# getanteon/alaz

Measured on AMD Instinct MI355X. Metric: L7 edge-events/s ingested->scored service-map, higher is better.
Workload: dtype u64; 1 GPU; C3 device-resident replay: 10000 pods / 5000 services / 1000000 edges, 10000000 HTTP l7 events per window already in HBM, 2-layer SAGE + MLP score, partitioned K1 (variant 0, 8-byte records, 512 partitions); 2-batch HBM ring (value excludes PCIe: see end_to_end with --full); events_per_window=10000000, layers=2, windows_in_flight=1, parallelism=1 GPU

## Files before the change

### alaz_amd/csrc/servicegraph.hip

```cpp
#include <hip/hip_runtime.h>
#include <hip/hip_ext.h>

#include <algorithm>
#include <cmath>
#include <cstdio>
#include <cstring>
#include <chrono>
#include <condition_variable>
#include <thread>
#include <mutex>
#include <string>
#include <unordered_map>
#include <vector>

#include <dlfcn.h>

#include "join_host.hpp"
#include "sg_plan.hpp"
#include "sg_kernels.h"
#include "sg_sel.h"
#include "sg_trend.h"
#include "sg_node_trend.h"
#include "sg_rank.h"
#include "sg_incident.h"
// ... 141 lines not shown
                    u32* blk = nullptr; u32* stage = nullptr; u32* stage_idx = nullptr; std::vector<sg_group_edge*> rows; std::vector<u64*> count;
                    std::vector<u32*> row_group, perm; std::vector<char> valid; hipEvent_t ev = nullptr; bool pending = false;
                    std::vector<u32> h_map; u32* h_up = nullptr; hipEvent_t up_ev = nullptr; bool up_pending = false; u32 dirty_lo = 0, dirty_hi = 0;
                    u32 hi_group = 0; } grp;
    Baseline<sg_edge_trend> gtrend;
    Vanished gvanished;
    IdxSel<sg_group_edge> gsel;
    Rollup<sgplan::GroupNodesPlan> gnodes;
    Baseline<sg_node_trend> gntrend;
    NSel gnsel;
    Rank<sgplan::GroupRankPlan> grank;
    Incidents<sgplan::GroupIncidentPlan> ginc;
};

namespace {

sg_engine::WinSlot& work(sg_engine* e) { return e->slots[e->cur]; }
int ran_slot(const sg_engine* e) { return e->last.slot >= 0 ? e->last.slot : e->cur; }
sg_engine::WinSlot& ran(sg_engine* e) { return e->slots[ran_slot(e)]; }

#define HIP_TRY(e, call)                                                                       \
    do {                                                                                       \
        hipError_t _r = (call);                                                                \
        if (_r != hipSuccess) {                                                                \
            (e)->err = std::string(#call) + ": " + hipGetErrorString(_r);                      \
            return _r == hipErrorOutOfMemory ? SG_ENOMEM : SG_ENODEV;                          \
        }                                                                                      \
    } while (0)

template <typename T>
int dev_alloc(sg_engine* e, T** p, size_t n, int fill = 0) {
    void* q = nullptr;
    size_t bytes = std::max<size_t>(n, 1) * sizeof(T);
    constexpr size_t kArenaMax = (size_t)32 << 20, kArenaChunk = (size_t)256 << 20, kArenaAlign = 4096;
    if (e->plan.arena_on && bytes < kArenaMax) {
        const size_t need = (bytes + kArenaAlign - 1) & ~(kArenaAlign - 1);
        if (need > e->arena_left) {
            void* c = nullptr;
            HIP_TRY(e, hipMalloc(&c, kArenaChunk));
            e->allocs.push_back(c);
            e->arena_base = static_cast<char*>(c); e->arena_left = kArenaChunk;
        }
        q = e->arena_base; e->arena_base += need; e->arena_left -= need;
    } else {
        HIP_TRY(e, hipMalloc(&q, bytes));
        e->allocs.push_back(q);
    }
    HIP_TRY(e, hipMemsetAsync(q, fill, bytes, e->slots[0].stream));
    *p = (T*)q;
    return SG_OK;
}

hipStream_t pick(sg_engine* e, void* s) { return s ? (hipStream_t)s : work(e).stream; }
hipStream_t pick_ran(sg_engine* e, void* s) { return s ? (hipStream_t)s : e->last.slot >= 0 ? e->last.stream : work(e).stream; }

hipEvent_t get_event(sg_engine* e) {
    if (!e->ev_pool.empty()) { hipEvent_t v = e->ev_pool.back(); e->ev_pool.pop_back(); return v; }
    hipEvent_t v; hipEventCreate(&v); return v;
}

struct Timed {
    sg_engine* e; hipStream_t s; TimingRec r; bool on;
    Timed(sg_engine* e_, hipStream_t s_, int kernel) : e(e_), s(s_), on(e_ && ((e_->timing >> kernel) & 1u)) {
        if (on) { r.kernel = kernel; r.a = get_event(e); r.b = get_event(e); hipEventRecord(r.a, s); }
    }
    ~Timed() { if (on) { hipEventRecord(r.b, s); e->trecs.push_back(r); } }
};

static_assert(sgplan::kK1bWarmU == K1B_WARM_U, "sg_plan.hpp's copy of pass B's warm U");
constexpr int k4_threads(int fi, bool proj, bool split) { return split ? (proj ? 512 : 256) : (fi == 32 ? 1024 : 512); }
template <class FnT, const auto& Keys> struct Family { typedef FnT Fn; static constexpr auto& keys = Keys; };
struct K1aWide : Family<K1aFn, sgplan::kK1aWideKeys> { template <size_t I> static Fn at() { constexpr auto k = keys[I]; return k1a_partition<(bool)k[0], (bool)k[1], (bool)k[2]>; } };
struct K1aTile : Family<K1aFn, sgplan::kK1aTileKeys> { template <size_t I> static Fn at() { constexpr auto k = keys[I]; return k1a_tile_partition<k[0], (bool)k[1], k[2]>; } };
struct K1aTeam : Family<K1aFn, sgplan::kK1aTeamKeys> { template <size_t I> static Fn at() { constexpr auto k = keys[I]; return k1a_team_partition<k[0], (bool)k[1], 2, 1024, k[2]>; } };
struct K1bMerge : Family<K1bFn, sgplan::kK1bMergeKeys> { template <size_t I> static Fn at() {
    constexpr auto k = keys[I]; if constexpr (k[2]) return k1b_merge<k[0], (bool)k[1]>; else return k1b_merge_wide<k[0], (bool)k[1]>; } };
struct K1bStream : Family<K1bFn, sgplan::kK1bStreamKeys> { template <size_t I> static Fn at() {
    constexpr auto k = keys[I]; if constexpr (k[4]) return k1b_stream_merge<k[0], k[1], (bool)k[2], k[3]>; else return k1b_stream_merge_wide<k[0], k[1], (bool)k[2], k[3]>; } };
struct K4Layer : Family<K4LayerFn, sgplan::kK4LayerKeys> { template <size_t I> static Fn at() {
    constexpr auto k = keys[I]; return k4_sage_layer<k[0], (bool)k[1], (bool)k[2], k4_threads(k[0], k[2], k[3]), (bool)k[3]>; } };
constexpr K2RowptrFn kK2Rowptr[2] = {k2_rowptr<K2_RP_ROWS, false>, k2_rowptr<K2_RP_ROWS_DH, true>};
constexpr K4GatherFn kK4Gather[2] = {k4_gather<32>, k4_gather<64>};
constexpr K5ProjFn kK5Proj[2] = {k5_node_proj<false>, k5_node_proj<true>};
constexpr K5ScoreFn kK5Score[2] = {k5_edge_score<false>, k5_edge_score<true>};
template <class F, size_t... I>
const std::array<typename F::Fn, sizeof...(I)>& kernel_table(std::index_sequence<I...>) {
    static const std::array<typename F::Fn, sizeof...(I)> t{{F::template at<I>()...}};
    return t;
}
template <class F> const auto& kernel_table() { return kernel_table<F>(std::make_index_sequence<F::keys.size()>{}); }
template <class F, class... A>
typename F::Fn kernel_of(bool& ok, A... args) {
    const int i = sgplan::find_key(F::keys, sgplan::Key<sizeof...(A)>{{(int)args...}});
    if (i < 0) ok = false;
    return i < 0 ? nullptr : kernel_table<F>()[i];
}
template <class... K>
hipError_t lds_limit(size_t bytes, K... kernels) {
    for (const void* f : {reinterpret_cast<const void*>(kernels)...}) {
        const hipError_t r = hipFuncSetAttribute(f, hipFuncAttributeMaxDynamicSharedMemorySize, (int)bytes);
        if (r != hipSuccess) return r;
    }
    return hipSuccess;
}
template <class F>
hipError_t lds_limit_all(size_t bytes) { hipError_t r = hipSuccess; for (const auto f : kernel_table<F>()) if (r == hipSuccess) r = lds_limit(bytes, f); return r; }

int plan_pass_a(sg_engine* e) {
    sgplan::PassA pa = e->pa;
    if (!sgplan::plan_pass_a(e->plan, e->jt.l1_entries, e->jt.blocks_bytes(), e->ov, &pa)) { e->err = "K1 pass A: the join tables' level 1 and the piece counters do not fit a CU's LDS (fewer partitions / IP blocks needed)"; return SG_ENOSPC; }
    const sgplan::PassAKernel k = sgplan::choose_pass_a(e->plan, pa, e->cfg);
    bool ok = true;
    const K1aFn f = k.family == sgplan::K1A_TEAM ? kernel_of<K1aTeam>(ok, k.l2, k.sharded, k.pb)
                  : k.family == sgplan::K1A_TILE ? kernel_of<K1aTile>(ok, k.l2, k.sharded, k.nsub) : kernel_of<K1aWide>(ok, k.l2, k.sharded, k.hist);
    if (!ok) { e->err = "K1 pass A: the library holds no kernel for family " + std::to_string(k.family) + ", level 2 mode " + std::to_string(k.l2); return SG_ENODEV; }
    e->pa = pa; e->kn.k1a = k; e->fn.k1a = f;
    return SG_OK;
}
int resolve_kernels(sg_engine* e) {
    const sgplan::Kernels& k = e->kn;
    sg_engine::Fns& f = e->fn;
    bool ok = true;
    if (k.k1b_family == sgplan::K1B_STREAM) {
        f.k1b = kernel_of<K1bStream>(ok, k.k1b_u, k.k1b_spt, k.k1b_pack, 0, k.k1b_share);
        if (k.k1b_warm) f.k1b_try = kernel_of<K1bStream>(ok, sgplan::kK1bWarmU, k.k1b_spt, k.k1b_pack, 1, k.k1b_share);
        if (k.k1b_warm) f.k1b_cold = kernel_of<K1bStream>(ok, sgplan::kK1bWarmU, k.k1b_spt, k.k1b_pack, 2, k.k1b_share);
    } else if (k.k1b_family == sgplan::K1B_MERGE) f.k1b = kernel_of<K1bMerge>(ok, k.k1b_u, k.k1b_hist, k.k1b_share);
    f.k2_rowptr = kK2Rowptr[k.k2_dh]; f.k5_proj = kK5Proj[k.k5_mfma];
    for (int w = 0; w < 2; w++) for (int pj = 0; pj < 2; pj++) f.k4_layer[w][pj] = kernel_of<K4Layer>(ok, w ? 64 : 32, k.k4_mfma, pj, k.k4_split);
    if (!ok) { e->err = "the library holds no kernel for one of the plan's choices (sg_plan.hpp choose_kernels)"; return SG_ENODEV; }
    return SG_OK;
}


void join_view(const sg_engine* e, Dev& d) {
    d.jl1mask = e->jt.l1_entries - 1;
    d.jl2_words = e->jt.use_blocks ? e->jt.blocks_used * 256u : 0u;
    d.ck_n = e->jt.ck_n;
    d.jstage_bytes = (u32)((size_t)e->jt.l1_entries * 8 + (e->pa.l2_in_lds ? e->jt.blocks_bytes() : 0));
    d.jl2_in_lds = e->pa.l2_in_lds ? 1u : 0u;
    d.k1a_ct = e->pa.k1a_ct;
}

int sync_tables(sg_engine* e, hipStream_t s) {
    sgjoin::Table& jt = e->jt;
    if (!jt.need_full && jt.dirty.empty()) return SG_OK;
    for (hipStream_t ks : e->k1_streams) if (ks != s) { HIP_TRY(e, hipEventRecord(e->k1_ev, ks)); HIP_TRY(e, hipStreamWaitEvent(s, e->k1_ev, 0)); }
    e->k1_streams.clear();
    if (jt.rebuilds == 0 && !jt.rebuild()) { e->err = "join table build failed: raise max_ips"; return SG_ENOSPC; }
    if (jt.need_full) {
        HIP_TRY(e, hipEventSynchronize(e->blob_ev));
        std::memcpy(e->h_blob, jt.blob, (size_t)jt.L.words * 4);
        HIP_TRY(e, hipMemcpyAsync(e->d_blob, e->h_blob, (size_t)jt.L.words * 4, hipMemcpyHostToDevice, s));
        HIP_TRY(e, hipEventRecord(e->blob_ev, s));
        jt.uploaded_full();
        e->st.join_full_uploads++;
    } else {
        std::vector<std::pair<u32, u32>> log;
        jt.take_dirty(log);
        std::unordered_map<u32, u32> last;
        last.reserve(log.size() * 2);
        for (auto& kv : log) last[kv.first] = kv.second;
        const int slot = e->upd_next; e->upd_next = (slot + 1) % kUpdSlots;
        HIP_TRY(e, hipEventSynchronize(e->upd_ev[slot]));
        u32 n = 0;
        for (auto& kv : last) e->h_upd[slot][n++] = make_uint2(kv.first, kv.second);
        HIP_TRY(e, hipMemcpyAsync(e->d_upd[slot], e->h_upd[slot], (size_t)n * sizeof(uint2), hipMemcpyHostToDevice, s));
// ... 589 lines not shown
    a.groups = e->grp.rows[e->cur]; a.gcount = e->grp.count[e->cur];
    a.max_groups = P.max_groups; a.gk = (u32)P.gk; a.hi_group = e->grp.hi_group; a.nc = P.nc;
    return a;
}
int launch_group_nodes(sg_engine* e, hipStream_t s) {
    GroupNodesArgs a = group_nodes_view(e);
    return launch_rollup(e, e->gnodes, e->gnodes.plan, s, a, a.nd, k16_out, k16_in_part, k16_count, k16_write);
}
static_assert(sgplan::kGrpRankThreads == K17_THREADS && sgplan::kGrpRankRangeRows == K17_NR && sgplan::kGrpRankMaxWgs == K17_MAX_WGS &&
              sgplan::kGrpRankNodeRows == K17_NODE_ROWS && K17_THREADS % K17_NODE_ROWS == 0 &&
              2 * sgplan::kGrpRankRangeRows * 8 <= sgplan::kLdsBytes, "plan_group_rank sizes the launches of sg_group_rank.h");
int launch_group_rank(sg_engine* e, hipStream_t s) {
    const sgplan::GroupRankPlan& P = e->grank.plan;
    GroupRankArgs a{};
    a.g = group_nodes_view(e);
    a.pos_wgs = P.pos_wgs; a.pos = e->grank.pos; a.w = e->grank.w;
    return launch_ranking(e, workload_space(e), P, s, a, [&](dim3 nt) {
        hipLaunchKernelGGL(k17_pos, dim3(P.pos_wgs), nt, 0, s, a);
        hipLaunchKernelGGL(k17_prep, dim3(P.prep_wgs), nt, 0, s, a);
    }, k17_edge<true>, k17_node<true, false>, k17_edge<false>, k17_node<false, false>, k17_node<false, true>);
}
void free_group_rank(sg_engine* e) { free_stage(e->grank); }
static_assert(sgplan::kGrpIncThreads == K18_THREADS && sgplan::kGrpIncMaxWgs == K18_MAX_WGS && sgplan::kGrpIncSlots == K12_SLOTS &&
              sgplan::kIncKeysBytes == sizeof(K12Keys), "plan_group_incidents sizes the launches of sg_group_incident.h");
int launch_group_incidents(sg_engine* e, hipStream_t s) {
    const sgplan::GroupIncidentPlan& P = e->ginc.plan;
    GroupIncArgs a{};
    a.g = group_nodes_view(e);
    a.pos = e->ginc.pos; a.esrc = e->ginc.esrc;
    return launch_grouping(e, workload_space(e), P, s, a, a.g.nd, P.fold_wgs, k18_init, k18_hook, k18_label, k18_number, k18_nodes, k18_rows, k18_finish);
}
void free_group_incidents(sg_engine* e) { free_stage(e->ginc); }
template <class Row>
void free_idxsel(sg_engine::IdxSel<Row>& s) {
    if (s.mem || s.h_n) hipDeviceSynchronize();
    if (s.mem) hipFree(s.mem);
    if (s.h_n) hipHostFree(s.h_n);
    if (s.ev) hipEventDestroy(s.ev);
    s = sg_engine::IdxSel<Row>{};
}
void free_group_nodes(sg_engine* e) {
    free_group_incidents(e);
    free_group_rank(e);
    free_idxsel(e->gnsel);
    free_baseline(e->gntrend);
    free_stage(e->gnodes);
}

void free_groups(sg_engine* e) {
    free_group_nodes(e);
    free_edge_trend(group_edge_space(e));
    sg_engine::Groups& x = e->grp;
    if (x.mem) hipDeviceSynchronize();
    if (x.h_up) hipHostFree(x.h_up);
    if (x.up_ev) hipEventDestroy(x.up_ev);
    free_stage(x);
}

void free_incidents(sg_engine* e) {
    free_tracks(e);
    free_stage(e->inc);
}

void free_nodes(sg_engine* e) {
    free_incidents(e);
    free_rank(e);
    free_baseline(e->ntrend);
    free_stage(e->nodes);
}

void drop_incidents(sg_engine* e, const EdgeSpace& es) {
    const NodeSpace ns = es.nodes(e);
    if (ns.inc->on && ns.inc->p.by != SG_SEL_SCORE) ns.inc_off(e);
}

int do_score(sg_engine* e, hipStream_t s, bool proj_done, bool fuse_reset, bool* did_reset) {
    const Dev& d = work(e).d;
    if (!e->have_w) { e->err = "sg_load_weights not called"; return SG_ESTATE; }
    const float* Wh = e->d_W + layer_offset(e->cfg.layers);
    const bool fr = fuse_reset && d.variant == 0;
    {
        Timed t(e, s, 5);
        if (!(proj_done && d.world == 1)) hipLaunchKernelGGL(e->fn.k5_proj, dim3(grid_for(d.ncap, 16)), dim3(256), 0, s, d, d.h[e->cfg.layers], Wh);
        hipLaunchKernelGGL(kK5Score[fr], dim3((int)e->plan.k5_grid), dim3(256), 0, s, d, Wh);
    }
    if (did_reset) *did_reset = fr;
    HIP_TRY(e, hipGetLastError());
    if (const int rc = note_w_read(e, s)) return rc;
    if (e->trend.on) { const int rc = launch_trend(e, s); if (rc) return rc; }
    if (e->nodes.on) {
        if (const int rc = launch_nodes(e, s)) return rc;
        if (e->ntrend.on) { if (const int rc = launch_node_trend(e, node_space(e), s, k10_count, k10_write)) return rc; }
        if (e->rank.on) { if (const int rc = launch_rank(e, s)) return rc; }
        if (e->inc.on) { if (const int rc = launch_incidents(e, s)) return rc; }
        if (e->trk.on) { if (const int rc = launch_tracks(e, s)) return rc; }
    }
    if (e->grp.on) {
        if (const int rc = launch_groups(e, s)) return rc;
        if (e->gtrend.on) { if (const int rc = launch_group_trend(e, s)) return rc; }
        if (e->gnodes.on) {
            if (const int rc = launch_group_nodes(e, s)) return rc;
            if (e->gntrend.on) { if (const int rc = launch_node_trend(e, workload_space(e), s, k16_tcount, k16_twrite)) return rc; }
            if (e->grank.on) { if (const int rc = launch_group_rank(e, s)) return rc; }
            if (e->ginc.on) { if (const int rc = launch_group_incidents(e, s)) return rc; }
        }
    }
    return SG_OK;
}

int do_reset(sg_engine* e, hipStream_t s) {
    sg_engine::WinSlot& w = work(e);
    hipLaunchKernelGGL(k_reset_window, dim3(grid_for(std::max<u64>((u64)w.d.ncap * SG_NODE_STAT_SUM_WORDS, e->plan.obcap), 256, 512)), dim3(256), 0, s, w.d);
    HIP_TRY(e, hipGetLastError());
    w.closed = false;
    w.events_in = 0;
    return SG_OK;
}

void window_timed_end(sg_engine* e, hipStream_t s) {
    if (!e->win_ta) return;
    TimingRec r; r.kernel = 10; r.a = e->win_ta; r.b = get_event(e);
    hipEventRecord(r.b, s);
    e->trecs.push_back(r);
    e->win_ta = nullptr;
}

void account_window(sg_engine* e) {
    sg_engine::WinSlot& w = work(e);
    const size_t E = (size_t)e->h_ctr[C_N_EDGES];
    sg_stats& st = e->st;
    st.windows++;
    st.last_window_events = e->h_ctr[C_N_EVENTS];
    st.last_window_edges = E;
    st.last_window_nodes = e->h_ctr[C_N_NODES];
    st.events_dropped_src += e->h_ctr[C_DROPPED_SRC];
    st.events_dropped_cap += e->h_ctr[C_DROPPED_CAP];
    st.events_misrouted += e->h_ctr[C_MISROUTED];
    {
        const u64 h = e->h_ctr[C_HALO_OVF];
        st.halo_overflow += h - w.halo_ovf_seen;
        w.halo_ovf_seen = h;
    }
    st.alive_in += e->h_ctr[C_ALIVE_SEEN];
    st.alive_dropped += e->h_ctr[C_ALIVE_DROPPED];
    st.last_window_new_edges = 0;
    if (w.d.warm && w.plain) st.windows_plain++;
    else if (w.d.warm) {
        const bool cold = e->h_ctr[C_LAST_COLD] != 0;
        if (cold) st.windows_cold++; else st.windows_warm++;
        if (!cold && e->h_ctr[C_LAST_DELTA]) { st.windows_delta++; st.last_window_new_edges = e->h_ctr[C_LAST_DELTA]; }
    }
    if (e->h_ctr[C_N_EVENTS]) {
        st.last_window_tmin_ms = (int64_t)((e->first_user - (e->first_kernel - e->h_ctr[C_TMIN_NS])) / 1000000ull);
        st.last_window_tmax_ms = (int64_t)((e->first_user - (e->first_kernel - e->h_ctr[C_TMAX_NS])) / 1000000ull);
    } else { st.last_window_tmin_ms = st.last_window_tmax_ms = 0; }
}

int view_reserve(sg_engine* e, size_t E) {
    if (E <= e->h_rows_cap) return SG_OK;
    if (e->h_rows_old) { hipHostFree(e->h_rows_old); e->h_rows_old = nullptr; }
    e->h_rows_old = e->h_rows; e->h_rows = nullptr; e->h_rows_cap = 0;
    const size_t want = std::min<size_t>(next_pow2(std::max<size_t>(E, 1024)), std::max<size_t>(e->cfg.max_edges, E));
    HIP_TRY(e, hipHostMalloc((void**)&e->h_rows, want * sizeof(sg_edge_out)));
    e->h_rows_cap = want;
    return SG_OK;
}
int do_read(sg_engine* e, sg_edge_out* out, size_t cap, size_t* n, const sg_edge_out** view = nullptr) {
// ... 2219 lines not shown
```

### alaz_amd/csrc/sg_k5.h

```cpp
#pragma once

template <bool USE_MFMA>
__global__ __launch_bounds__(256) void k5_node_proj(Dev d, const float* __restrict__ hL, const float* __restrict__ Wh) {
    constexpr int LDA = SG_F_HID + 2;
    __shared__ float A[16 * LDA];
    __shared__ u32 vid[16];
    const bool listed = d.world > 1 && d.ctr[C_ACT_L] != SG_ACT_NONE;
    const u32 N = listed ? (u32)d.ctr[C_ACT_P] : (u32)d.ctr[C_N_NODES];
    const float* __restrict__ Wu = Wh; const float* __restrict__ Wv = Wh + SG_F_HID * SG_F_HID;
    const float* __restrict__ b1 = Wv + SG_F_HID * SG_F_HID + SG_F_EDGE * SG_F_HID;
    const u32 wave = threadIdx.x >> 6, lane = threadIdx.x & 63;
    for (u32 tile = blockIdx.x; tile * 16 < N; tile += gridDim.x) {
        const u32 v0 = tile * 16;
        if (threadIdx.x < 16) vid[threadIdx.x] = v0 + threadIdx.x < N ? (listed ? d.act_p[v0 + threadIdx.x] : v0 + threadIdx.x) : 0u;
        __syncthreads();
        for (u32 idx = threadIdx.x; idx < 16 * SG_F_HID; idx += 256) {
            const u32 r = idx >> 6, k = idx & 63;
            A[r * LDA + k] = (v0 + r < N) ? hL[(size_t)vid[r] * SG_F_HID + k] : 0.0f;
        }
        __syncthreads();
        if (USE_MFMA) {
            const int jb = wave * 16, i = lane & 15;
            const float bj = b1[jb + i];
            f32x4 p = { bj, bj, bj, bj }, q = { 0.0f, 0.0f, 0.0f, 0.0f };
            p = dense_tile_mfma<SG_F_HID>(A, LDA, Wu, jb, p);
            q = dense_tile_mfma<SG_F_HID>(A, LDA, Wv, jb, q);
#pragma unroll
            for (int r = 0; r < 4; r++) {
                const u32 row = (lane >> 4) * 4 + r;
                if (v0 + row < N) { d.P[(size_t)vid[row] * SG_F_HID + SG_PQ_POS(jb + i)] = p[r]; d.Q[(size_t)vid[row] * SG_F_HID + SG_PQ_POS(jb + i)] = q[r]; }
            }
        } else {
            const u32 row = threadIdx.x >> 4, jq = (threadIdx.x & 15) * 4;
            float p[4], q[4];
#pragma unroll
            for (int c = 0; c < 4; c++) { p[c] = b1[jq + c]; q[c] = 0.0f; }
            for (int k = 0; k < (int)SG_F_HID; k++) {
                const float a = A[row * LDA + k];
#pragma unroll
                for (int c = 0; c < 4; c++) { p[c] = fmaf(a, Wu[(size_t)k * SG_F_HID + jq + c], p[c]); q[c] = fmaf(a, Wv[(size_t)k * SG_F_HID + jq + c], q[c]); }
            }
            if (v0 + row < N)
#pragma unroll
                for (int c = 0; c < 4; c++) { d.P[(size_t)vid[row] * SG_F_HID + SG_PQ_POS(jq + c)] = p[c]; d.Q[(size_t)vid[row] * SG_F_HID + SG_PQ_POS(jq + c)] = q[c]; }
        }
        __syncthreads();
    }
}

static_assert(sizeof(sg_edge_out) == 64 && offsetof(sg_edge_out, sum_ns) == 0 && offsetof(sg_edge_out, max_ns) == 8 && offsetof(sg_edge_out, sumsq_us) == 16 &&
              offsetof(sg_edge_out, from_ref) == 24 && offsetof(sg_edge_out, to_ref) == 28 && offsetof(sg_edge_out, count) == 32 && offsetof(sg_edge_out, err_count) == 36 &&
              offsetof(sg_edge_out, score) == 40 && offsetof(sg_edge_out, lat_z) == 44 && offsetof(sg_edge_out, err_ratio) == 48 && offsetof(sg_edge_out, alive) == 52 &&
              offsetof(sg_edge_out, p50_us) == 56 && offsetof(sg_edge_out, p99_us) == 60, "k5_edge_score writes a row as eight 8-byte words");
template <bool RESET>
__global__ __launch_bounds__(256) __attribute__((amdgpu_waves_per_eu(3))) void k5_edge_score(Dev d, const float* __restrict__ Wh) {
    const u32 E = (u32)d.ctr[C_N_EDGES], nk = (u32)d.ctr[C_N_KNOWN], nl = (u32)d.ctr[C_N_LABELS];
    const float* __restrict__ We = Wh + 2 * SG_F_HID * SG_F_HID;
    const float* __restrict__ w2 = We + SG_F_EDGE * SG_F_HID + SG_F_HID;
    const float b2 = w2[SG_F_HID];
    const u32 lane = threadIdx.x & 63, q = lane & 15, g = lane >> 4;
    const u32 wave = (blockIdx.x * 256 + threadIdx.x) >> 6, nw = (gridDim.x * 256) >> 6;
    float we[SG_F_EDGE][4], w2r[4];
#pragma unroll
    for (int m = 0; m < 4; m++) {
        w2r[m] = w2[q + 16 * m];
#pragma unroll
        for (int k = 0; k < (int)SG_F_EDGE; k++) we[k][m] = We[k * SG_F_HID + q + 16 * m];
    }
    auto step = [&](const float4 P4, const float4 Q4, const float (&ek)[SG_F_EDGE]) -> float {
        const float pq[4] = {P4.x + Q4.x, P4.y + Q4.y, P4.z + Q4.z, P4.w + Q4.w};
        float r[4];
#pragma unroll
        for (int m = 0; m < 4; m++) {
            float x = pq[m];
#pragma unroll
            for (int k = 0; k < (int)SG_F_EDGE; k++) x = fmaf(ek[k], we[k][m], x);
            x = x > 0.0f ? x : 0.0f;
            r[m] = x * w2r[m];
        }
        float sum = (r[0] + r[2]) + (r[1] + r[3]);
        sum = sum + xor_partner_f32(sum, 8); sum = sum + xor_partner_f32(sum, 4);
        sum = sum + xor_partner_f32(sum, 2); sum = sum + xor_partner_f32(sum, 1);
        return sum;
    };
    static_assert(SG_F_EDGE == 8, "k5_edge_score spreads two 8-float edge feature vectors over a DPP row of 16 lanes");
    const u32* __restrict__ idsrc = (q & 1u) ? d.col : d.csr_from;
    const u32 wk = lane & 7u, we8 = lane >> 3;
    const u32* __restrict__ srcA = wk == 3 ? d.csr_from : reinterpret_cast<const u32*>(d.errr);
    const u32* __restrict__ srcB = wk == 3 ? d.col : (wk == 5 ? reinterpret_cast<const u32*>(d.latz) : d.alive_csr);
    const u32 accj = wk < 3 ? wk + 1 : 0u;
    const int srcl = (int)(((we8 & 3u) << 4) | (we8 < 4 ? 0u : 8u));
    if (E) {
        const u32 stride = nw * 8, last = E - 1;
        u32 pa = wave * 8 + g, pb = pa + 4;
        struct K5Set { float4 PA, QA, PB, QB; u32 ew, wa, wb; u64 wacc; };
        auto ids_of = [&](u32 xa, u32 xb) -> u32 { const u32 px = (q & 2u) ? xb : xa; return idsrc[px < E ? px : last]; };
        auto issue = [&](u32 idw_, u32 xa, u32 xb, u32 x0, K5Set& S) {
            u32 ua = dpp32b<0x150>(idw_), va = dpp32b<0x151>(idw_), ub = dpp32b<0x152>(idw_), vb = dpp32b<0x153>(idw_);
            if SG_ABL(d, 0x1000u) { ua &= 15u; va &= 15u; ub &= 15u; vb &= 15u; }
            const u32 ca = xa < E ? xa : last, cb = xb < E ? xb : last;
            S.PA = reinterpret_cast<const float4*>(d.P + (size_t)ua * SG_F_HID)[q]; S.QA = reinterpret_cast<const float4*>(d.Q + (size_t)va * SG_F_HID)[q];
            S.PB = reinterpret_cast<const float4*>(d.P + (size_t)ub * SG_F_HID)[q]; S.QB = reinterpret_cast<const float4*>(d.Q + (size_t)vb * SG_F_HID)[q];
            S.ew = __float_as_uint(d.efeat[(size_t)(q < 8 ? ca : cb) * SG_F_EDGE + (q & 7u)]);
            const u32 er_ = x0 + we8, ec_ = er_ < E ? er_ : last;
            S.wacc = d.acc_csr[(size_t)ec_ * 4 + accj];
            S.wa = srcA[ec_]; S.wb = srcB[ec_];
        };
        auto iter = [&](K5Set& cur, K5Set& nxt, const u32 idw_next, u32& idw_after, const u32 p0) {
            const u32 na = pa + stride, nb = pb + stride;
            idw_after = ids_of(na + stride, nb + stride);
            issue(idw_next, na, nb, p0 + stride, nxt);
            __builtin_amdgcn_sched_barrier(0);
            const float4 PA = cur.PA, QA = cur.QA, PB = cur.PB, QB = cur.QB;
            const u32 ew = cur.ew, wa = cur.wa, wb = cur.wb; const u64 wacc = cur.wacc;
            const u32 er = p0 + we8, ec = er < E ? er : last;
            const float eka[SG_F_EDGE] = {__uint_as_float(dpp32b<0x150>(ew)), __uint_as_float(dpp32b<0x151>(ew)), __uint_as_float(dpp32b<0x152>(ew)), __uint_as_float(dpp32b<0x153>(ew)),
                                          __uint_as_float(dpp32b<0x154>(ew)), __uint_as_float(dpp32b<0x155>(ew)), __uint_as_float(dpp32b<0x156>(ew)), __uint_as_float(dpp32b<0x157>(ew))};
            const float ekb[SG_F_EDGE] = {__uint_as_float(dpp32b<0x158>(ew)), __uint_as_float(dpp32b<0x159>(ew)), __uint_as_float(dpp32b<0x15A>(ew)), __uint_as_float(dpp32b<0x15B>(ew)),
                                          __uint_as_float(dpp32b<0x15C>(ew)), __uint_as_float(dpp32b<0x15D>(ew)), __uint_as_float(dpp32b<0x15E>(ew)), __uint_as_float(dpp32b<0x15F>(ew))};
            const float sa = step(PA, QA, eka);
            const float sb = step(PB, QB, ekb);
            const float mysum = __shfl(q < 8 ? sa : sb, srcl, 64);
            u64 val = wacc;
            if (wk == 3) val = (u64)ref_of_dense(wa, nk, nl) | ((u64)ref_of_dense(wb, nk, nl) << 32);
            else if (wk == 5) { const float logit = mysum + b2; val = (u64)__float_as_uint(1.0f / (1.0f + expf(-logit))) | ((u64)wb << 32); }
            else if (wk == 6) val = (u64)wa | ((u64)wb << 32);
            else if (wk == 7) {
                val = 0;
                if (d.hist) {
                    const ulonglong2* __restrict__ ac = reinterpret_cast<const ulonglong2*>(d.acc_csr + (size_t)ec * 4);
                    const u32 count = (u32)(ac[0].x & 0xFFFFFFFFull); const u64 max_ns = ac[1].x;
                    if (count) {
                        const uint4* hp = reinterpret_cast<const uint4*>(d.hist_csr + (size_t)ec * SG_HIST_BINS);
                        const uint4 h0 = hp[0], h1 = hp[1], h2 = hp[2], h3 = hp[3];
                        const u32 hb[SG_HIST_BINS] = {h0.x, h0.y, h0.z, h0.w, h1.x, h1.y, h1.z, h1.w, h2.x, h2.y, h2.z, h2.w, h3.x, h3.y, h3.z, h3.w};
                        u64 r50 = ((u64)count * 50 + 99) / 100, r99 = ((u64)count * 99 + 99) / 100;
                        r50 = r50 ? r50 : 1; r99 = r99 ? r99 : 1;
                        u64 cum = 0; u32 b50 = SG_HIST_BINS - 1, b99 = SG_HIST_BINS - 1; bool f50 = false, f99 = false;
#pragma unroll
                        for (u32 b = 0; b < SG_HIST_BINS; b++) { cum += hb[b]; if (!f50 && cum >= r50) { b50 = b; f50 = true; } if (!f99 && cum >= r99) { b99 = b; f99 = true; } }
                        u64 e50 = b50 == SG_HIST_BINS - 1 ? max_ns : (1ull << (17 + b50)), e99 = b99 == SG_HIST_BINS - 1 ? max_ns : (1ull << (17 + b99));
                        e50 = e50 > max_ns ? max_ns : e50; e99 = e99 > max_ns ? max_ns : e99;
                        e50 /= 1000ull; e99 /= 1000ull;
                        val = (u64)(e50 > 0xFFFFFFFFull ? 0xFFFFFFFFu : (u32)e50) | ((u64)(e99 > 0xFFFFFFFFull ? 0xFFFFFFFFu : (u32)e99) << 32);
                    }
                }
            }
            {
                const u32 p0u = (u32)__builtin_amdgcn_readfirstlane((int)p0);
                const u32 nrow = SG_ABL(d, 0x2000u) ? 0u : (E - p0u < 8u ? E - p0u : 8u);
                const __amdgpu_buffer_rsrc_t rr_ = __builtin_amdgcn_make_buffer_rsrc(reinterpret_cast<u64*>(d.rows) + (size_t)p0u * 8, 0, (int)(nrow * 64u), 0x00020000);
                v2u_t dv; dv.x = (u32)val; dv.y = (u32)(val >> 32);
                __builtin_amdgcn_raw_buffer_store_b64(dv, rr_, lane * 8u, 0, 0);
            }
            pa = na; pb = nb;
        };
        K5Set A, B;
        u32 i1 = ids_of(pa + stride, pb + stride), i2;
        { const u32 id0 = ids_of(pa, pb); issue(id0, pa, pb, wave * 8, A); }
        for (u32 p0 = wave * 8; p0 < E; p0 += 2 * stride) {
            iter(A, B, i1, i2, p0);
            if (p0 + stride >= E) break;
            iter(B, A, i2, i1, p0 + stride);
        }
    }
    if (RESET) {
        const u64 tid = (u64)blockIdx.x * 256 + threadIdx.x, nt = (u64)gridDim.x * 256;
        const u64 nc = (u64)d.ncap + 1;
        if (!d.dh_g) for (u64 i = tid; i < nc * SG_DEG_REP; i += nt) { d.deg[i * SG_DEG_STRIDE] = 0; if (d.warm) d.deg2[i * SG_DEG_STRIDE] = 0; }
        for (u64 i = tid; i < nc; i += nt) d.cursor[i] = 0;
        for (u64 i = tid; i < (u64)d.ncap * SG_NODE_STAT_SUM_WORDS; i += nt) d.st_sum[i] = 0;
        for (u64 i = tid; i < (u64)d.ncap * SG_NODE_STAT_MAX_WORDS; i += nt) d.st_max[i] = 0;
        for (u64 i = tid; i <= d.obmask; i += nt) d.obkeys[i] = 0;
        if (tid == 0) { d.ctr[C_COLD] = 0; d.ctr[C_DELTA_N] = 0; d.ctr[C_OB_RAW] = 0; }
    }
}
```

### alaz_amd/csrc/sg_plan.hpp

```cpp
#pragma once
#include <algorithm>
#include <array>
#include <cmath>
#include <cstdint>
#include <cstdlib>
#include <cstring>
#include <initializer_list>
#include <optional>
#include <string>
#include <vector>

#include "../../include/servicegraph.h"
#include "sg_sizes.h"

namespace sgplan {

typedef uint32_t u32;
typedef uint64_t u64;

constexpr size_t kLdsBytes = 160 * 1024;
constexpr int kStageSlots = 32;
constexpr size_t kPrepareLds = 4096;

inline u32 next_pow2(u64 v) { u64 p = 1; while (p < v) p <<= 1; return (u32)p; }
// ... 881 lines not shown
    plan_rollup(n, max_edges, n.gk, n.nc, kGrpNodesMaxInWgs, slots);
    return n;
}
inline int check_group_node_trend(const sg_trend_params& p, u32 nc, sg_trend_params* out) { return check_node_trend(p, nc, out); }
using GroupNodeTrendPlan = TrendPlan;
inline TrendPlan plan_group_node_trend(u32 nc, u32 slots, const sg_trend_params& p) {
    return plan_baseline(p, 2 * (u64)nc, std::max<u64>(nc, 1) * sizeof(sg_node_trend), slots);
}
inline NodeSelPlan plan_group_node_select(u32 nc, u64 counter_bytes) { return plan_node_select(nc, counter_bytes); }

constexpr u32 kGrpRankThreads = 256, kGrpRankRangeRows = 8192, kGrpRankSliceEdges = 2048, kGrpRankMaxSlices = 256, kGrpRankMaxWgs = 1024,
              kGrpRankNodeRows = 32;
constexpr u64 kGrpRankPartBudget = 128ull << 20;
static_assert(kGrpRankMaxWgs == kRankMaxWgs, "plan_rank_block sizes the seed sums of both rankings");
struct GroupRankPlan : RankBlock {
    typedef unsigned long long Weight;
    u32 nc = 0;
    u64 gk = 0;
    u32 pos_wgs = 0;
    u64 pos_bytes = 0;
    u64 edge_bytes = 0;
    u64 w_bytes = 0;
    u64 pos_off = 0, edge_off[2] = {}, w_off = 0;
};
inline u32 group_rank_live_wgs(const GroupRankPlan& r, u64 n) {
    return (u32)std::min<u64>(r.ranges, (n + kGrpRankRangeRows - 1) / kGrpRankRangeRows) * r.slices;
}
inline GroupRankPlan plan_group_rank(u64 max_edges, u32 nc, u64 gk, u32 slots) {
    GroupRankPlan r;
    const u64 ME = std::max<u64>(max_edges, 1), NC = std::max<u32>(nc, 1), GK = std::max<u64>(gk, 1);
    r.nc = nc; r.gk = gk;
    r.ranges = (u32)((NC + kGrpRankRangeRows - 1) / kGrpRankRangeRows);
    r.slices = (u32)std::max<u64>(1, std::min<u64>(kGrpRankMaxSlices, (ME + kGrpRankSliceEdges - 1) / kGrpRankSliceEdges));
    r.slices = (u32)std::max<u64>(1, std::min<u64>(r.slices, kGrpRankPartBudget / ((u64)r.ranges * kGrpRankRangeRows * 8)));
    r.pos_wgs = (u32)std::max<u64>(1, std::min<u64>(kGrpRankMaxWgs, (NC + kGrpRankThreads - 1) / kGrpRankThreads));
    r.prep_wgs = (u32)std::max<u64>(1, std::min<u64>(kGrpRankMaxWgs, (ME + 4 * kGrpRankThreads - 1) / (4 * kGrpRankThreads)));
    r.node_wgs = (u32)std::max<u64>(1, std::min<u64>(kGrpRankMaxWgs, (NC + kGrpRankNodeRows - 1) / kGrpRankNodeRows));
    r.pos_bytes = trend_align(GK * 4);
    r.edge_bytes = trend_align(ME * 4);
    r.w_bytes = trend_align(ME * 8);
    plan_rank_block(r, NC, kGrpRankRangeRows, slots, [&r](Block& b) {
        const char* const edge[2] = {"src", "dst"};
        r.pos_off = b.take("pos", r.pos_bytes);
        for (int k = 0; k < 2; k++) r.edge_off[k] = b.take(edge[k], r.edge_bytes);
        r.w_off = b.take("w", r.w_bytes);
    });
    return r;
}

constexpr u32 kGrpIncThreads = 256, kGrpIncMaxWgs = 1024, kGrpIncMaxRowWgs = 256, kGrpIncFoldRounds = 8, kGrpIncSlots = 512;
static_assert(kGrpIncThreads == kIncThreads && kGrpIncMaxWgs == kIncMaxWgs && kGrpIncMaxRowWgs == kIncMaxRowWgs,
              "plan_incident_block sizes the grids of both groupings");
struct GroupIncidentPlan : IncidentBlock {
    u32 nc = 0;
    u64 gk = 0;
    u32 fold_wgs = 0;
    u64 pos_bytes = 0;
    u64 node_bytes = 0;
    u64 esrc_bytes = 0;
    u64 pos_off = 0, node_off[4] = {}, esrc_off = 0;
};
inline u64 group_incident_fold_rows(const GroupIncidentPlan& r, u64 n) { return (n + r.fold_wgs - 1) / r.fold_wgs; }
inline u64 group_incident_row_edges(const GroupIncidentPlan& r, u64 g) { return (g + r.row_wgs - 1) / r.row_wgs; }
inline GroupIncidentPlan plan_group_incidents(u64 max_edges, u32 nc, u64 gk, u32 slots) {
    GroupIncidentPlan r;
    const u64 ME = std::max<u64>(max_edges, 1), NC = std::max<u32>(nc, 1), GK = std::max<u64>(gk, 1);
    r.nc = nc; r.gk = gk;
    const u64 fold_rows = (u64)kGrpIncFoldRounds * kGrpIncThreads;
    r.fold_wgs = (u32)std::max<u64>(1, std::min<u64>(kGrpIncMaxWgs, (NC + fold_rows - 1) / fold_rows));
    r.pos_bytes = trend_align(GK * 4);
    r.node_bytes = trend_align(NC * 4);
    r.esrc_bytes = trend_align(ME * 4);
    plan_incident_block(r, max_edges, NC, slots, [&r](Block& b) {
        const char* const node[4] = {"parent", "flag", "lab", "num"};
        r.pos_off = b.take("pos", r.pos_bytes);
        for (int k = 0; k < 4; k++) r.node_off[k] = b.take(node[k], r.node_bytes);
        r.esrc_off = b.take("esrc", r.esrc_bytes);
    });
    return r;
}

inline bool close_folds(const Plan& p, bool warm, bool warm_try, u32 ob_mode) { return p.prepare_fold && warm && warm_try && ob_mode == 1u; }

template <class D>
void plan_to_dev(const Plan& p, const sg_config& cfg, D& d) {
    d.max_known = cfg.max_known_nodes; d.max_labels = cfg.max_labels; d.max_obip = p.max_obip;
    d.rank = cfg.rank; d.world = cfg.world; d.max_edges = cfg.max_edges; d.layers = cfg.layers;
    d.ncap = p.ncap; d.emask = p.ecap - 1; d.obmask = p.obcap - 1;
    d.variant = p.variant; d.narrow = p.narrow; d.hist = p.hist; d.agg_slots = p.agg_slots;
    d.nb = p.nb; d.np = p.np; d.pb = p.pb; d.rb = p.rb; d.nwg = p.nwg; d.k1b_split = p.k1b_split; d.npb = p.npb; d.k1b_ht = p.k1b_ht;
    d.pcap = p.pcap; d.sa = p.sa; d.sn = p.sn; d.sw = p.sw; d.punits = p.punits; d.ss = p.ss; d.pslots = p.pslots; d.ovf_cap = p.ovf_cap;
    d.warm = p.warm; d.alive_cap = p.alive_cap; d.hub_cap = p.hub_cap;
    d.k2_sortw = p.k2_sortw; d.dh_g = p.dh_g; d.dh_ppw = p.dh_ppw; d.dh_ns = p.dh_ns;
    d.ablate = p.ablate;
}

}
```

Baseline: 23.23 billion events/s.

## Use buffer-resource loads and 32-bit gather offsets in k5 edge score

The edge-score kernel now reads per-edge ids, features, accumulators and weights through windowed raw buffer loads. Hardware range checks take the place of per-lane clamp-to-last index math, and the source/destination ids double as the wk==3 payload instead of being loaded twice. P/Q row gathers use 32-bit byte offsets (v<<8|q<<4) when ncap*256 fits in 32 bits, with a wide variant selected on the host otherwise. The edge-feature FMAs are packed into two-wide vector FMAs. This aims to cut address arithmetic, VGPR pressure and redundant loads, but adds scalar descriptor construction per iteration.

```diff
diff --git a/alaz_amd/csrc/servicegraph.hip b/alaz_amd/csrc/servicegraph.hip
--- a/alaz_amd/csrc/servicegraph.hip
+++ b/alaz_amd/csrc/servicegraph.hip
@@ -247,7 +247,8 @@
 constexpr K2RowptrFn kK2Rowptr[2] = {k2_rowptr<K2_RP_ROWS, false>, k2_rowptr<K2_RP_ROWS_DH, true>};
 constexpr K4GatherFn kK4Gather[2] = {k4_gather<32>, k4_gather<64>};
 constexpr K5ProjFn kK5Proj[2] = {k5_node_proj<false>, k5_node_proj<true>};
-constexpr K5ScoreFn kK5Score[2] = {k5_edge_score<false>, k5_edge_score<true>};
+constexpr K5ScoreFn kK5Score[2][2] = {{k5_edge_score<false>, k5_edge_score<true>},
+                                      {k5_edge_score_wide<false>, k5_edge_score_wide<true>}};
 template <class F, size_t... I>
 const std::array<typename F::Fn, sizeof...(I)>& kernel_table(std::index_sequence<I...>) {
     static const std::array<typename F::Fn, sizeof...(I)> t{{F::template at<I>()...}};
@@ -1003,7 +1004,7 @@
     {
         Timed t(e, s, 5);
         if (!(proj_done && d.world == 1)) hipLaunchKernelGGL(e->fn.k5_proj, dim3(grid_for(d.ncap, 16)), dim3(256), 0, s, d, d.h[e->cfg.layers], Wh);
-        hipLaunchKernelGGL(kK5Score[fr], dim3((int)e->plan.k5_grid), dim3(256), 0, s, d, Wh);
+        hipLaunchKernelGGL(kK5Score[!sgplan::k5_gather_fits32(d.ncap)][fr], dim3((int)e->plan.k5_grid), dim3(256), 0, s, d, Wh);
     }
     if (did_reset) *did_reset = fr;
     HIP_TRY(e, hipGetLastError());
diff --git a/alaz_amd/csrc/sg_k5.h b/alaz_amd/csrc/sg_k5.h
--- a/alaz_amd/csrc/sg_k5.h
+++ b/alaz_amd/csrc/sg_k5.h
@@ -52,14 +52,15 @@
               offsetof(sg_edge_out, from_ref) == 24 && offsetof(sg_edge_out, to_ref) == 28 && offsetof(sg_edge_out, count) == 32 && offsetof(sg_edge_out, err_count) == 36 &&
               offsetof(sg_edge_out, score) == 40 && offsetof(sg_edge_out, lat_z) == 44 && offsetof(sg_edge_out, err_ratio) == 48 && offsetof(sg_edge_out, alive) == 52 &&
               offsetof(sg_edge_out, p50_us) == 56 && offsetof(sg_edge_out, p99_us) == 60, "k5_edge_score writes a row as eight 8-byte words");
-template <bool RESET>
-__global__ __launch_bounds__(256) __attribute__((amdgpu_waves_per_eu(3))) void k5_edge_score(Dev d, const float* __restrict__ Wh) {
+template <bool RESET, bool WIDE>
+__device__ __forceinline__ void k5_edge_score_body(const Dev& d, const float* __restrict__ Wh) {
     const u32 E = (u32)d.ctr[C_N_EDGES], nk = (u32)d.ctr[C_N_KNOWN], nl = (u32)d.ctr[C_N_LABELS];
     const float* __restrict__ We = Wh + 2 * SG_F_HID * SG_F_HID;
     const float* __restrict__ w2 = We + SG_F_EDGE * SG_F_HID + SG_F_HID;
     const float b2 = w2[SG_F_HID];
     const u32 lane = threadIdx.x & 63, q = lane & 15, g = lane >> 4;
     const u32 wave = (blockIdx.x * 256 + threadIdx.x) >> 6, nw = (gridDim.x * 256) >> 6;
+    typedef float v2f_t __attribute__((ext_vector_type(2)));
     float we[SG_F_EDGE][4], w2r[4];
 #pragma unroll
     for (int m = 0; m < 4; m++) {
@@ -68,51 +69,63 @@
         for (int k = 0; k < (int)SG_F_EDGE; k++) we[k][m] = We[k * SG_F_HID + q + 16 * m];
     }
     auto step = [&](const float4 P4, const float4 Q4, const float (&ek)[SG_F_EDGE]) -> float {
-        const float pq[4] = {P4.x + Q4.x, P4.y + Q4.y, P4.z + Q4.z, P4.w + Q4.w};
-        float r[4];
+        v2f_t x01 = {P4.x + Q4.x, P4.y + Q4.y}, x23 = {P4.z + Q4.z, P4.w + Q4.w};
 #pragma unroll
-        for (int m = 0; m < 4; m++) {
-            float x = pq[m];
-#pragma unroll
-            for (int k = 0; k < (int)SG_F_EDGE; k++) x = fmaf(ek[k], we[k][m], x);
-            x = x > 0.0f ? x : 0.0f;
-            r[m] = x * w2r[m];
+        for (int k = 0; k < (int)SG_F_EDGE; k++) {
+            const v2f_t e2 = {ek[k], ek[k]};
+            x01 = __builtin_elementwise_fma(e2, v2f_t{we[k][0], we[k][1]}, x01); x23 = __builtin_elementwise_fma(e2, v2f_t{we[k][2], we[k][3]}, x23);
         }
+        const float r[4] = {__builtin_fmaxf(x01.x, 0.0f) * w2r[0], __builtin_fmaxf(x01.y, 0.0f) * w2r[1],
+                            __builtin_fmaxf(x23.x, 0.0f) * w2r[2], __builtin_fmaxf(x23.y, 0.0f) * w2r[3]};
         float sum = (r[0] + r[2]) + (r[1] + r[3]);
         sum = sum + xor_partner_f32(sum, 8); sum = sum + xor_partner_f32(sum, 4);
         sum = sum + xor_partner_f32(sum, 2); sum = sum + xor_partner_f32(sum, 1);
         return sum;
     };
     static_assert(SG_F_EDGE == 8, "k5_edge_score spreads two 8-float edge feature vectors over a DPP row of 16 lanes");
-    const u32* __restrict__ idsrc = (q & 1u) ? d.col : d.csr_from;
+    static_assert(SG_F_HID * sizeof(float) == 256, "k5_edge_score's gather offset is v << 8 | q << 4");
+    const u32 q16 = q << 4;
+    auto pq_row = [&](const float* __restrict__ base, u32 v) -> float4 {
+        if constexpr (WIDE) return reinterpret_cast<const float4*>(base + (size_t)v * SG_F_HID)[q];
+        else return *reinterpret_cast<const float4*>(reinterpret_cast<const char*>(base) + ((v << 8) | q16));
+    };
     const u32 wk = lane & 7u, we8 = lane >> 3;
-    const u32* __restrict__ srcA = wk == 3 ? d.csr_from : reinterpret_cast<const u32*>(d.errr);
-    const u32* __restrict__ srcB = wk == 3 ? d.col : (wk == 5 ? reinterpret_cast<const u32*>(d.latz) : d.alive_csr);
     const u32 accj = wk < 3 ? wk + 1 : 0u;
     const int srcl = (int)(((we8 & 3u) << 4) | (we8 < 4 ? 0u : 8u));
     if (E) {
         const u32 stride = nw * 8, last = E - 1;
-        u32 pa = wave * 8 + g, pb = pa + 4;
-        struct K5Set { float4 PA, QA, PB, QB; u32 ew, wa, wb; u64 wacc; };
-        auto ids_of = [&](u32 xa, u32 xb) -> u32 { const u32 px = (q & 2u) ? xb : xa; return idsrc[px < E ? px : last]; };
-        auto issue = [&](u32 idw_, u32 xa, u32 xb, u32 x0, K5Set& S) {
-            u32 ua = dpp32b<0x150>(idw_), va = dpp32b<0x151>(idw_), ub = dpp32b<0x152>(idw_), vb = dpp32b<0x153>(idw_);
+        const u32 w0 = (u32)__builtin_amdgcn_readfirstlane((int)(wave * 8));
+        auto window = [&](const void* base, u32 pos, u32 elem, u32 span) -> __amdgpu_buffer_rsrc_t {
+            const u32 n = pos < E ? (E - pos < span ? E - pos : span) : 0u;
+            return __builtin_amdgcn_make_buffer_rsrc(const_cast<char*>(reinterpret_cast<const char*>(base)) + (size_t)pos * elem, 0, (int)(n * elem), 0x00020000);
+        };
+        const u32 ge = (q & 2u) ? 4u + g : g;
+        const u32 off_id0 = ge * 4u;
+        const u32 off_id = wk == 3 ? we8 * 4u : (stride + ge) * 4u;
+        const u32 off_ef = ((q < 8 ? g : 4u + g) * SG_F_EDGE + (q & 7u)) * 4u;
+        const u32 off_acc = (we8 * 4u + accj) * 8u, off_w = we8 * 4u;
+        struct K5Ids { u32 f, t; };
+        struct K5Set { float4 PA, QA, PB, QB; u32 ew, werr, wlat, walv; v2u_t acc; };
+        auto ids_at = [&](u32 pos, u32 off, u32 span) -> K5Ids {
+            return {__builtin_amdgcn_raw_buffer_load_b32(window(d.csr_from, pos, 4, span), off, 0, 0), __builtin_amdgcn_raw_buffer_load_b32(window(d.col, pos, 4, span), off, 0, 0)};
+        };
+        auto issue = [&](const K5Ids& id, u32 pos, K5Set& S) {
+            u32 ua = dpp32b<0x150>(id.f), va = dpp32b<0x150>(id.t), ub = dpp32b<0x152>(id.f), vb = dpp32b<0x152>(id.t);
             if SG_ABL(d, 0x1000u) { ua &= 15u; va &= 15u; ub &= 15u; vb &= 15u; }
-            const u32 ca = xa < E ? xa : last, cb = xb < E ? xb : last;
-            S.PA = reinterpret_cast<const float4*>(d.P + (size_t)ua * SG_F_HID)[q]; S.QA = reinterpret_cast<const float4*>(d.Q + (size_t)va * SG_F_HID)[q];
-            S.PB = reinterpret_cast<const float4*>(d.P + (size_t)ub * SG_F_HID)[q]; S.QB = reinterpret_cast<const float4*>(d.Q + (size_t)vb * SG_F_HID)[q];
-            S.ew = __float_as_uint(d.efeat[(size_t)(q < 8 ? ca : cb) * SG_F_EDGE + (q & 7u)]);
-            const u32 er_ = x0 + we8, ec_ = er_ < E ? er_ : last;
-            S.wacc = d.acc_csr[(size_t)ec_ * 4 + accj];
-            S.wa = srcA[ec_]; S.wb = srcB[ec_];
+            S.PA = pq_row(d.P, ua); S.QA = pq_row(d.Q, va); S.PB = pq_row(d.P, ub); S.QB = pq_row(d.Q, vb);
+            S.ew = __builtin_amdgcn_raw_buffer_load_b32(window(d.efeat, pos, SG_F_EDGE * 4, 8), off_ef, 0, 0);
+            S.acc = __builtin_amdgcn_raw_buffer_load_b64(window(d.acc_csr, pos, 32, 8), off_acc, 0, 0);
+            S.werr = __builtin_amdgcn_raw_buffer_load_b32(window(d.errr, pos, 4, 8), off_w, 0, 0);
+            S.wlat = __builtin_amdgcn_raw_buffer_load_b32(window(d.latz, pos, 4, 8), off_w, 0, 0);
+            S.walv = __builtin_amdgcn_raw_buffer_load_b32(window(d.alive_csr, pos, 4, 8), off_w, 0, 0);
         };
-        auto iter = [&](K5Set& cur, K5Set& nxt, const u32 idw_next, u32& idw_after, const u32 p0) {
-            const u32 na = pa + stride, nb = pb + stride;
-            idw_after = ids_of(na + stride, nb + stride);
-            issue(idw_next, na, nb, p0 + stride, nxt);
+        auto iter = [&](K5Set& cur, K5Set& nxt, const K5Ids& idw_next, K5Ids& idw_after, const u32 p0) {
+            idw_after = ids_at(p0 + stride, off_id, stride + 8);
+            issue(idw_next, p0 + stride, nxt);
             __builtin_amdgcn_sched_barrier(0);
             const float4 PA = cur.PA, QA = cur.QA, PB = cur.PB, QB = cur.QB;
-            const u32 ew = cur.ew, wa = cur.wa, wb = cur.wb; const u64 wacc = cur.wacc;
+            const u32 ew = cur.ew, wa = wk == 3 ? idw_next.f : cur.werr, wb = wk == 3 ? idw_next.t : (wk == 5 ? cur.wlat : cur.walv);
+            const u64 wacc = (u64)cur.acc.x | ((u64)cur.acc.y << 32);
             const u32 er = p0 + we8, ec = er < E ? er : last;
             const float eka[SG_F_EDGE] = {__uint_as_float(dpp32b<0x150>(ew)), __uint_as_float(dpp32b<0x151>(ew)), __uint_as_float(dpp32b<0x152>(ew)), __uint_as_float(dpp32b<0x153>(ew)),
                                           __uint_as_float(dpp32b<0x154>(ew)), __uint_as_float(dpp32b<0x155>(ew)), __uint_as_float(dpp32b<0x156>(ew)), __uint_as_float(dpp32b<0x157>(ew))};
@@ -147,18 +160,14 @@
                 }
             }
             {
-                const u32 p0u = (u32)__builtin_amdgcn_readfirstlane((int)p0);
-                const u32 nrow = SG_ABL(d, 0x2000u) ? 0u : (E - p0u < 8u ? E - p0u : 8u);
-                const __amdgpu_buffer_rsrc_t rr_ = __builtin_amdgcn_make_buffer_rsrc(reinterpret_cast<u64*>(d.rows) + (size_t)p0u * 8, 0, (int)(nrow * 64u), 0x00020000);
                 v2u_t dv; dv.x = (u32)val; dv.y = (u32)(val >> 32);
-                __builtin_amdgcn_raw_buffer_store_b64(dv, rr_, lane * 8u, 0, 0);
+                __builtin_amdgcn_raw_buffer_store_b64(dv, window(d.rows, p0, 64, SG_ABL(d, 0x2000u) ? 0u : 8u), lane * 8u, 0, 0);
             }
-            pa = na; pb = nb;
         };
         K5Set A, B;
-        u32 i1 = ids_of(pa + stride, pb + stride), i2;
-        { const u32 id0 = ids_of(pa, pb); issue(id0, pa, pb, wave * 8, A); }
-        for (u32 p0 = wave * 8; p0 < E; p0 += 2 * stride) {
+        K5Ids i1 = ids_at(w0, off_id, stride + 8), i2;
+        { const K5Ids id0 = ids_at(w0, off_id0, 8); issue(id0, w0, A); }
+        for (u32 p0 = w0; p0 < E; p0 += 2 * stride) {
             iter(A, B, i1, i2, p0);
             if (p0 + stride >= E) break;
             iter(B, A, i2, i1, p0 + stride);
@@ -175,3 +184,7 @@
         if (tid == 0) { d.ctr[C_COLD] = 0; d.ctr[C_DELTA_N] = 0; d.ctr[C_OB_RAW] = 0; }
     }
 }
+template <bool RESET>
+__global__ __launch_bounds__(256) __attribute__((amdgpu_waves_per_eu(3))) void k5_edge_score(Dev d, const float* __restrict__ Wh) { k5_edge_score_body<RESET, false>(d, Wh); }
+template <bool RESET>
+__global__ __launch_bounds__(256) __attribute__((amdgpu_waves_per_eu(3))) void k5_edge_score_wide(Dev d, const float* __restrict__ Wh) { k5_edge_score_body<RESET, true>(d, Wh); }
diff --git a/alaz_amd/csrc/sg_plan.hpp b/alaz_amd/csrc/sg_plan.hpp
--- a/alaz_amd/csrc/sg_plan.hpp
+++ b/alaz_amd/csrc/sg_plan.hpp
@@ -987,6 +987,8 @@
 
 inline bool close_folds(const Plan& p, bool warm, bool warm_try, u32 ob_mode) { return p.prepare_fold && warm && warm_try && ob_mode == 1u; }
 
+inline bool k5_gather_fits32(u32 ncap) { return (u64)ncap * (SG_F_HID * sizeof(float)) < (1ull << 32); }
+
 template <class D>
 void plan_to_dev(const Plan& p, const sg_config& cfg, D& d) {
     d.max_known = cfg.max_known_nodes; d.max_labels = cfg.max_labels; d.max_obip = p.max_obip;
```

After: 23.33 billion events/s (median of 6 runs). Within noise of the previous version (+0.4%).
